# ZhenlongYuan/DVP-MVS

Measured on AMD Instinct MI355X. Metric: Mpixels/sec/PatchMatch-iteration, higher is better.
Workload: dtype f32

## Files before the change

__graft_entry__.py:

```python
import importlib
import os
import subprocess
import sys

ROOT = os.path.dirname(os.path.abspath(__file__))
if ROOT not in sys.path:
    sys.path.insert(0, ROOT)


def build() -> None:
    subprocess.check_call(["make", "-s", "-C", os.path.join(ROOT, "dvp-mvs_amd", "csrc")])
    host = os.path.join(ROOT, "dvp-mvs_amd", "host")
    if os.path.exists(os.path.join(host, "Makefile")):
        subprocess.check_call(["make", "-s", "-C", host])
    subprocess.check_call(["make", "-s", "-C", os.path.join(ROOT, "oracle")])
    subprocess.check_call(["make", "-s", "-C", os.path.join(ROOT, "tests", "emul")])
    subprocess.check_call(["make", "-s", "-C", os.path.join(ROOT, "tests", "host")])
    subprocess.check_call(["make", "-s", "-C", os.path.join(ROOT, "tests", "half16")])
    subprocess.check_call(["make", "-s", "-C", os.path.join(ROOT, "tests", "jpeg_host")])
    pkg = importlib.import_module("dvp-mvs_amd")
    lib = pkg.get_capi().lib()
    missing = [s for s in pkg.get_capi().EXPORTS if not hasattr(lib, s)]
    if missing:
        raise RuntimeError("libdvp_mvs_hip.so lacks symbols: %s" % missing)


def smoke() -> None:
    import numpy as np
    pkg = importlib.import_module("dvp-mvs_amd")
    synth, capi = pkg.synth, pkg.get_capi()
    from oracle import oracle as O
    W, H, S = 96, 64, 3
    sc = synth.make_scene(W, H, S)
    p = synth.default_params(S + 1, max_iterations=1, state=synth.FIRST_INIT, use_APD=0)
    p["depth_min"] = np.float32(2.5) * np.float32(0.6)
    p["depth_max"] = np.float32(6.5) * np.float32(1.2)
    state = dict(planes=np.zeros((H * W, 4), np.float32), edge=sc["edge"], label=sc["label"],
                 radius=np.full(H * W, 5, np.int32))
    g = capi.from_scene(sc, p, device=0)
    g.upload_state(**state)
    g.run_patchmatch()
    o = O.from_scene(sc, p)
    o.upload_state(**state)
    o.run_patchmatch()
    pg, po = g.get("planes"), o.get("planes")
    same = (pg.view(np.uint32) == po.view(np.uint32)) | (np.isnan(pg) & np.isnan(po))
    if not same.all():
        raise AssertionError("smoke: HIP planes differ from the oracle in %d values" % int((~same).sum()))
    for n in ("selected_views", "weak_info", "radius"):
# ... 10 lines not shown
```

dvp-mvs_amd/csrc/dvp_engine.hip:

```cpp
#include "dvp_stages.hpp"
#include "dvp_jpeg_enc.h"
#include <hip/hip_runtime.h>
#include <cstdlib>
#include <string>
#include <vector>
#include <cstdio>
#include <cstring>
#include <mutex>
#include <condition_variable>
#include <thread>
#include <chrono>
#include <algorithm>
#include <cmath>

using namespace dvp;

struct LaunchArgs {
	int tiles_x, tiles, rows, half, colour, iter;
};

template <int STAGE, int SMP, int MV = 32>
__device__ __forceinline__ void stage_body(const Dev& d, const LaunchArgs& a) {
	const int lane = threadIdx.x & 63;
	const int wave = threadIdx.x >> 6;
// ... 131 lines not shown
	}
	const int off = incl - n;
	const int total = __shfl(incl, 63, 64);
	{
		int k = 0;
		for (uint32_t m = uniq; m; m &= m - 1, ++k) items[off + k] = (uint8_t)lane;
	}
	__syncthreads();
	unsigned long long cnt = 0;
	for (int i0 = 0; i0 < total; i0 += 64) {
		const bool valid = i0 + lane < total;
		const int i = valid ? i0 + lane : total - 1;
		const int pl = items[i];
		const int k = i - __shfl(off, pl, 64);
		uint32_t m = (uint32_t)__shfl((int)uniq, pl, 64);
		for (int j = 0; j < k; ++j) m &= m - 1;
		const int slot = dvp_ctz(m);
		PatchCtx ci;
		ci.tab = PatchTab{&lds_tab[pl], 64};
		ci.sum_ref = __shfl(c.sum_ref, pl, 64);
		ci.sum_ref_ref = __shfl(c.sum_ref_ref, pl, 64);
		ci.wsum = __shfl(c.wsum, pl, 64);
		ci.radius = __shfl(c.radius, pl, 64);
		ci.inc = __shfl(c.inc, pl, 64);
		ci.fast = __shfl(c.fast, pl, 64);
		const int ipx = __shfl(px, pl, 64), ipy = __shfl(py, pl, 64);
		strong_eval_item<SMP>(d, ci, ipx, ipy, slot, valid, d.eval_counter ? &cnt : nullptr);
	}
	if (d.eval_counter && cnt) atomicAdd(d.eval_counter, cnt);
}
extern "C" __global__ void __launch_bounds__(64, DVP_LB_HEAVY) dvp_strong_eval_items(const Dev d, const LaunchArgs a) { strong_eval_items_body<0>(d, a); }
extern "C" __global__ void __launch_bounds__(64, DVP_LB_HEAVY) dvp_strong_eval_items_exact(const Dev d, const LaunchArgs a) { strong_eval_items_body<1>(d, a); }
DVP_KERNEL64(dvp_strong_refine, kStageStrongRefine, DVP_LB_HEAVY)
DVP_KERNEL64(dvp_strong_refine_lanes, kStageStrongRefineLanes, DVP_LB_HEAVY)
template <int MV>
__device__ __forceinline__ void strong_decide_body(const Dev& d, const LaunchArgs& a) {
	int px, py;
	if (!block_to_pixel(blockIdx.x, threadIdx.x & 63, threadIdx.x >> 6, a.tiles_x, a.tiles, a.rows, a.half, a.colour, d.width, d.height, &px, &py)) return;
	if (d.weak_info[px + py * d.width] != DVP_WEAK) strong_decide_px<MV>(d, px, py, a.iter);
}
#ifndef DVP_LB_DECIDE
#define DVP_LB_DECIDE 4
#endif
#define DVP_DECIDE_KERNEL(MV) extern "C" __global__ void __launch_bounds__(256, DVP_LB_DECIDE) dvp_strong_decide_v##MV(const Dev d, const LaunchArgs a) { strong_decide_body<MV>(d, a); }
DVP_DECIDE_KERNEL(4)
DVP_DECIDE_KERNEL(6)
DVP_DECIDE_KERNEL(8)
DVP_DECIDE_KERNEL(10)
DVP_DECIDE_KERNEL(12)
DVP_DECIDE_KERNEL(16)
DVP_KERNEL(dvp_get_depth_normal, DVP_ST_GET_DEPTH_NORMAL, 1)
DVP_KERNEL(dvp_filter_strong, DVP_ST_FILTER_STRONG, 1)
DVP_KERNEL(dvp_depth_to_weak, DVP_ST_DEPTH_TO_WEAK, DVP_LB_HEAVY)
DVP_KERNEL(dvp_local_refine, DVP_ST_LOCAL_REFINE, DVP_LB_HEAVY)
DVP_KERNEL(dvp_depth_to_weak_refine, kStageSweeps, DVP_LB_HEAVY)
template <int WHAT>
__device__ __forceinline__ void sweep_light_body(const Dev& d, const LaunchArgs& a) {
	int px, py;
	if (!block_to_pixel(blockIdx.x, threadIdx.x & 63, threadIdx.x >> 6, a.tiles_x, a.tiles, a.rows, 0, 0, d.width, d.height, &px, &py)) return;
	if (WHAT != 0 && d.sweep_row1 > 0 && (py < d.sweep_row0 || py >= d.sweep_row1)) return;
	if (WHAT == 0) sweep_prepare_px(d, px, py);
	else if (WHAT == 1) sweep_decide1_px(d, px, py);
	else sweep_decide2_px(d, px, py);
}
extern "C" __global__ void __launch_bounds__(256) dvp_sweep_prepare(const Dev d, const LaunchArgs a) { sweep_light_body<0>(d, a); }
extern "C" __global__ void __launch_bounds__(256) dvp_sweep_decide1(const Dev d, const LaunchArgs a) { sweep_light_body<1>(d, a); }
extern "C" __global__ void __launch_bounds__(256) dvp_sweep_decide2(const Dev d, const LaunchArgs a) { sweep_light_body<2>(d, a); }
// ... 744 lines not shown
	size_t L = 0;
	hipStream_t stream = nullptr;
	int cand_mask_mode = -1;
	bool cand_mask_on = true;
	uint8_t* cand_mask = nullptr;
	unsigned *cand_list = nullptr, *cand_n = nullptr;
	uint32_t* sel_snap = nullptr;
	hipStream_t side = nullptr;
	hipEvent_t side_fork = nullptr, side_join = nullptr;
	Dev d{};
	std::vector<void*> allocs;
	float* images = nullptr;
	uint8_t* images8 = nullptr;
	int* images8_flag = nullptr;
	bool images8_ok = false;
	bool no_images8 = false;
	uint32_t* images16 = nullptr;
	bool images16_ok = false;
	bool no_images16 = false;
	float* image_stage = nullptr;
	float* depths = nullptr;
	uint32_t* edge_bits = nullptr;
	uint32_t* strong_bits = nullptr;
	uint32_t* strong_bits_t = nullptr;
	int* edge_sat = nullptr;
	DvpCamera* cameras = nullptr; ViewConst* views = nullptr; int* sector_taps = nullptr; int* sector_start = nullptr;
	f4* planes = nullptr; f4* planes_snap = nullptr; f4* fit_planes = nullptr;
	int* search_pos = nullptr;
	float* slot_costs = nullptr;
	float* strong_rec = nullptr;
	bool strong_split = true;
	bool eval_items = true;
	bool refine_lanes = true;
	f4* sweep_rec = nullptr; float* sweep_cost = nullptr; float* sweep_pc = nullptr;
	bool ransac_wave = false;
	bool sweep_split = true;
	bool sweep_force = false;
	double sweep_band_gb = 0.0;
	int sweep_band_rows = 0;
	bool gn_wave = false;
	float* costs = nullptr; float* costs_snap = nullptr; float* complex_ = nullptr;
	uint32_t* selected_views = nullptr;
	uint8_t* view_weight = nullptr; uint8_t* weak_info = nullptr; uint8_t* weak_reliable = nullptr; uint8_t* edge = nullptr;
	s2* label_stop = nullptr; s2* weak_nearest_strong = nullptr; s2* neighbours = nullptr; s2* gn_points = nullptr; int* gn_count = nullptr; s2* candidate = nullptr; s2* edge_neigh = nullptr; s2* label_boundary = nullptr;
	int* neighbours_map = nullptr; int* label = nullptr; int* radius = nullptr;
	unsigned long long* eval_counter = nullptr;
	float* scratch_out = nullptr;
	size_t weak_alloc = 0;
	AnchorRec* anchor_tab = nullptr;
	size_t anchor_tab_alloc = 0;
	bool anchor_tab_valid = false;
	bool anchor_tab_off = false;
	WeakRec* weak_rec = nullptr; f2* weak_ctab = nullptr; float* weak_ev = nullptr;
	size_t weak_phase_alloc = 0;
	bool weak_phased = true;
	int weak_phased_min = 8192;
	int weak_run[4] = { 64, 256, 1024, 1024 };
	int weak_group[4] = { 1, 4, 4, 2 };
	int* weak_list = nullptr;
	size_t weak_list_alloc = 0;
	int* weak_counts = nullptr;
	int* weak_totals_host = nullptr;
	uint8_t* coarse = nullptr;
	uint8_t* maps_out = nullptr;
	hipStream_t copy = nullptr;
	uint8_t* maps_host = nullptr;
// ... 77 lines not shown

static int ensure_images16(dvp_ctx* c) {
	if (c->images16) return 0;
	return dalloc(c, &c->images16, img16_plane_bytes(c->W, c->H) / 4 * c->NI, false);
}

static int set_device(dvp_ctx* c) {
	HIP_TRY(c, hipSetDevice(c->device));
	return 0;
}

extern "C" {

int dvp_ctx_create(int device, int width, int height, int num_images, dvp_ctx** out) {
	if (!out) return 1;
	*out = nullptr;
	if (width <= 0 || height <= 0 || num_images < 2 || num_images > DVP_MAX_IMAGES || width > 32767 || height > 32767) {
		g_create_error = "dvp_ctx_create: bad dimensions (2 <= num_images <= 32, sizes <= 32767: short2 pixel coordinates)";
		return 1;
	}
	{
		const unsigned long long pitch = ((unsigned long long)width + 2 * kImgPad + 63) / 64 * 64;
		if (pitch * ((unsigned long long)height + 2 * kImgPad) * 8ull >= (1ull << 32)) {
			g_create_error = "dvp_ctx_create: image too large (a padded row-pair plane must stay below 4 GiB)";
			return 1;
		}
	}
	dvp_ctx* c = new dvp_ctx();
	c->device = device; c->W = width; c->H = height; c->NI = num_images;
	c->no_images8 = getenv("DVP_NO_IMAGES8") != nullptr;
	c->no_images16 = getenv("DVP_NO_IMAGES16") != nullptr;
	if (const char* e = getenv("DVP_STRONG_SPLIT")) c->strong_split = atoi(e) != 0;
	if (const char* e = getenv("DVP_REFINE_LANES")) c->refine_lanes = atoi(e) != 0;
	if (const char* e = getenv("DVP_EVAL_ITEMS")) c->eval_items = atoi(e) != 0;
	if (const char* e = getenv("DVP_SWEEP_SPLIT")) { c->sweep_split = atoi(e) != 0; c->sweep_force = atoi(e) == 2; }
	if (const char* e = getenv("DVP_SWEEP_BAND_GB")) c->sweep_band_gb = atof(e);
	if (const char* e = getenv("DVP_WEAK_ANCHOR_TAB")) c->anchor_tab_off = atoi(e) == 0;
	if (const char* e = getenv("DVP_GN_WAVE")) c->gn_wave = atoi(e) != 0;
	if (const char* e = getenv("DVP_RANSAC_WAVE")) c->ransac_wave = atoi(e) != 0;
	if (const char* e = getenv("DVP_CAND_MASK")) c->cand_mask_mode = atoi(e) != 0 ? 1 : 0;
	if (const char* e = getenv("DVP_WEAK_PHASED")) c->weak_phased = atoi(e) != 0;
	if (const char* e = getenv("DVP_WEAK_PHASED_MIN")) c->weak_phased_min = atoi(e);
	if (const char* e = getenv("DVP_WEAK_RUNS")) {
		int g[4];
		if (sscanf(e, "%d,%d,%d,%d", &g[0], &g[1], &g[2], &g[3]) == 4)
			for (int i = 0; i < 4; ++i) c->weak_run[i] = g[i] < 1 ? 1 : g[i];
	}
	if (const char* e = getenv("DVP_WEAK_GROUPS")) {
		int g[4];
		if (sscanf(e, "%d,%d,%d,%d", &g[0], &g[1], &g[2], &g[3]) == 4)
			for (int i = 0; i < 4; ++i) c->weak_group[i] = g[i] < 1 ? 1 : (g[i] > kGrp ? kGrp : g[i]);
	}
	c->pitch = (width + 2 * kImgPad + 63) / 64 * 64;
	c->L = (size_t)width * height;
	auto fail = [&](int) { g_create_error = c->error; dvp_ctx_destroy(c); return 1; };
	if (set_device(c)) return fail(0);
	if (hipStreamCreateWithFlags(&c->stream, hipStreamNonBlocking) != hipSuccess) { c->error = "hipStreamCreate failed"; return fail(0); }
	if (hipStreamCreateWithFlags(&c->side, hipStreamNonBlocking) != hipSuccess || hipEventCreateWithFlags(&c->side_fork, hipEventDisableTiming) != hipSuccess ||
	    hipEventCreateWithFlags(&c->side_join, hipEventDisableTiming) != hipSuccess) { c->error = "hipStreamCreate failed"; return fail(0); }
	const size_t L = c->L, S = (size_t)num_images - 1, plane = (size_t)c->pitch * (height + 2 * kImgPad);
	int r = 0;
	r |= dalloc(c, &c->images, plane * num_images * 2);
	r |= dalloc(c, &c->images8, (size_t)img8_tiles_x(width) * img8_tiles_y(height) * 128 * num_images);
	r |= dalloc(c, &c->images8_flag, (size_t)1);
	r |= dalloc(c, &c->image_stage, plane * num_images);
	r |= dalloc(c, &c->cameras, (size_t)num_images);
// ... 44 lines not shown
int dvp_ctx_destroy(dvp_ctx* c) {
	if (!c) return 0;
	(void)hipSetDevice(c->device);
	{
		int limit_s = 120;
		if (const char* e = getenv("DVP_DOWNLOAD_WAIT_S")) limit_s = atoi(e);
		std::unique_lock<std::mutex> lk(c->dl_m);
		c->dl_cv.wait_for(lk, std::chrono::seconds(limit_s > 0 ? limit_s : 1), [c] { return !c->dl_busy; });
		c->dl_cv.wait(lk, [c] { return !c->dl_fetching; });
	}
	if (c->copy) { (void)hipStreamSynchronize(c->copy); (void)hipStreamDestroy(c->copy); }
	if (c->pv_copy) { (void)hipStreamSynchronize(c->pv_copy); (void)hipStreamDestroy(c->pv_copy); }
	if (c->stream) (void)hipStreamSynchronize(c->stream);
	for (auto& e : c->pv_enc) dvpjpeg::encoder_free(e);
	if (c->pv_total) (void)hipHostFree(c->pv_total);
	if (c->pv_done) (void)hipEventDestroy(c->pv_done);
	if (c->maps_host) (void)hipHostFree(c->maps_host);
	if (c->stream) (void)hipStreamSynchronize(c->stream);
	for (auto& e : c->events) { (void)hipEventDestroy(e.a); (void)hipEventDestroy(e.b); }
	for (void* p : c->allocs) (void)hipFree(p);
	if (c->weak_totals_host) (void)hipHostFree(c->weak_totals_host);
	if (c->side) { (void)hipStreamSynchronize(c->side); (void)hipStreamDestroy(c->side); }
	if (c->side_fork) (void)hipEventDestroy(c->side_fork);
	if (c->side_join) (void)hipEventDestroy(c->side_join);
	if (c->stream) (void)hipStreamDestroy(c->stream);
	delete c;
	return 0;
}

#ifndef DVP_BUILD_ID
#define DVP_BUILD_ID "unknown"
#endif
const char* dvp_build_id(void) { return DVP_BUILD_ID; }

struct FinishError { const dvp_ctx* c = nullptr; std::string msg; };
static thread_local FinishError t_finish_error;
const char* dvp_last_error(const dvp_ctx* c) {
	if (c && t_finish_error.c == c && !t_finish_error.msg.empty()) return t_finish_error.msg.c_str();
	return c ? c->error.c_str() : g_create_error.c_str();
}

static int upload_planes(dvp_ctx* c, float* dst, const float* const* src, int pitch_floats, hipMemcpyKind kind, float* pairs = nullptr) {
	if (set_device(c)) return 1;
	if (pitch_floats < c->W) { c->error = "pitch_floats < width"; return 1; }
	const size_t stride = (size_t)c->pitch * (c->H + 2 * kImgPad);
	for (int i = 0; i < c->NI; ++i) {
		if (!src[i]) { c->error = "null image pointer"; return 1; }
		HIP_TRY(c, hipMemcpy2DAsync(dst + (size_t)i * stride + (size_t)kImgPad * c->pitch + kImgPad, (size_t)c->pitch * 4, src[i],
		                            (size_t)pitch_floats * 4, (size_t)c->W * 4, (size_t)c->H, kind, c->stream));
	}
	{
		const long long cells = (long long)(2 * kImgPad * (c->W + 2 * kImgPad) + 2 * kImgPad * c->H) * c->NI;
		hipLaunchKernelGGL(dvp_pad_replicate, dim3((unsigned)((cells + 255) / 256)), dim3(256), 0, c->stream, dst, c->W, c->H, c->pitch, stride, c->NI);
		HIP_TRY(c, hipGetLastError());
	}
	if (pairs) {
		const int PH = c->H + 2 * kImgPad;
		hipLaunchKernelGGL(dvp_interleave_rows, dim3((unsigned)((c->pitch + 255) / 256), (unsigned)PH, (unsigned)c->NI), dim3(256), 0, c->stream,
		                   dst, pairs, PH, c->pitch, stride, c->NI);
		HIP_TRY(c, hipGetLastError());
		HIP_TRY(c, hipMemsetAsync(c->images8_flag, 0, sizeof(int), c->stream));
		const int t8x = img8_tiles_x(c->W), t8y = img8_tiles_y(c->H);
		const size_t n = (size_t)t8x * t8y * 64 * c->NI;
		hipLaunchKernelGGL(dvp_pairs_to_tiles, dim3((unsigned)((n + 255) / 256)), dim3(256), 0, c->stream, pairs, c->images8, c->W + 2 * kImgPad, PH, c->pitch, stride,
		                   t8x, t8y, c->NI, c->images8_flag);
		HIP_TRY(c, hipGetLastError());
// ... 465 lines not shown
		HIP_TRY(c, hipGetLastError());
	}
	if (stage == DVP_ST_GEN_EDGE_INFORM && c->d.params.use_label && c->d.weak_count > 0) {
		if (!c->label_stop) {
			if (dalloc(c, &c->label_stop, c->L * 8, false)) return 1;
			sync_dev_struct(c);
		}
		hipLaunchKernelGGL(dvp_edge_rays, dim3((c->W + c->H + 255) / 256, 8), dim3(256), 0, c->stream, c->d, 1);
		HIP_TRY(c, hipGetLastError());
	}
	switch (stage) {
	case DVP_ST_GEN_EDGE_INFORM:
		if (!fused) {
			if (gen_candidates_all_views(c->d)) hipLaunchKernelGGL(dvp_gen_candidates_views, dim3(g.grid(), (unsigned)((c->NI - 1 + kCandGroup - 1) / kCandGroup)), block, 0, c->stream, c->d, a);
			else hipLaunchKernelGGL(dvp_gen_candidates, dim3(g.grid(), (unsigned)(c->NI - 1)), block, 0, c->stream, c->d, a);
		}
		hipLaunchKernelGGL(c->d.sampler ? dvp_gen_edge_inform_exact : dvp_gen_edge_inform, grid, block, 0, c->stream, c->d, a);
		break;
	case DVP_ST_RANDOM_INIT: hipLaunchKernelGGL(c->d.sampler ? dvp_random_init_exact : dvp_random_init, grid, block, 0, c->stream, c->d, a); break;
	case DVP_ST_STRONG_UPDATE:
		if (c->strong_split && c->NI - 1 <= 16) {
			ensure_strong_split_buffers(c);
		}
		if (c->strong_split && c->NI - 1 <= 16) {
			const int S = c->NI - 1;
			if (c->eval_items) hipLaunchKernelGGL(c->d.sampler ? dvp_strong_eval_items_exact : dvp_strong_eval_items, wave_grid, wave_block, 0, c->stream, c->d, a);
			else hipLaunchKernelGGL(c->d.sampler ? dvp_strong_eval_exact : dvp_strong_eval, wave_grid, wave_block, 0, c->stream, c->d, a);
			if (S <= 4) hipLaunchKernelGGL(dvp_strong_decide_v4, grid, block, 0, c->stream, c->d, a);
			else if (S <= 6) hipLaunchKernelGGL(dvp_strong_decide_v6, grid, block, 0, c->stream, c->d, a);
			else if (S <= 8) hipLaunchKernelGGL(dvp_strong_decide_v8, grid, block, 0, c->stream, c->d, a);
			else if (S <= 10) hipLaunchKernelGGL(dvp_strong_decide_v10, grid, block, 0, c->stream, c->d, a);
			else if (S <= 12) hipLaunchKernelGGL(dvp_strong_decide_v12, grid, block, 0, c->stream, c->d, a);
			else hipLaunchKernelGGL(dvp_strong_decide_v16, grid, block, 0, c->stream, c->d, a);
			if (c->refine_lanes && (size_t)c->pitch * (c->H + 2 * kImgPad) * 8 * c->NI < ((size_t)1 << 32))
				hipLaunchKernelGGL(c->d.sampler ? dvp_strong_refine_lanes_exact : dvp_strong_refine_lanes, wave_grid, wave_block, 0, c->stream, c->d, a);
			else hipLaunchKernelGGL(c->d.sampler ? dvp_strong_refine_exact : dvp_strong_refine, wave_grid, wave_block, 0, c->stream, c->d, a);
		}
		else if (c->NI - 1 <= kNarrowViews) hipLaunchKernelGGL(c->d.sampler ? dvp_strong_update_v8_exact : dvp_strong_update_v8, grid, block, 0, c->stream, c->d, a);
		else if (c->NI - 1 <= 16) hipLaunchKernelGGL(c->d.sampler ? dvp_strong_update_v16_exact : dvp_strong_update_v16, grid, block, 0, c->stream, c->d, a);
		else hipLaunchKernelGGL(c->d.sampler ? dvp_strong_update_exact : dvp_strong_update, grid, block, 0, c->stream, c->d, a);
		break;
	case DVP_ST_GET_DEPTH_NORMAL: hipLaunchKernelGGL(c->d.sampler ? dvp_get_depth_normal_exact : dvp_get_depth_normal, grid, block, 0, c->stream, c->d, a); break;
	case DVP_ST_FILTER_STRONG: hipLaunchKernelGGL(c->d.sampler ? dvp_filter_strong_exact : dvp_filter_strong, grid, block, 0, c->stream, c->d, a); break;
	case DVP_ST_DEPTH_TO_WEAK: {
		const bool sweep_passes = fused && c->sweep_split && (c->d.params.geom_consistency || c->sweep_force);
		if (sweep_passes) ensure_sweep_buffers(c);
		if (sweep_passes && c->sweep_split) {
			const bool ex = c->d.sampler != 0;
			LaunchArgs s0 = a, s1 = a, sb = a;
			s0.iter = 0; s1.iter = 1; sb.iter = kSweepBorderOnly;
			const int etx = (c->W + 63) / 64, ety = (c->H + kSweepRows - 1) / kSweepRows;
			s0.tiles_x = s1.tiles_x = etx; s0.tiles = s1.tiles = etx * ety;
			const dim3 egrid((unsigned)(etx * ety), (unsigned)(c->NI - 1));
			hipLaunchKernelGGL(dvp_sweep_prepare, grid, block, 0, c->stream, c->d, a);
			const int band_rows = c->sweep_band_rows > 0 ? c->sweep_band_rows : c->H;
			for (int row0 = 0; row0 < c->H; row0 += band_rows) {
				Dev db = c->d;
				LaunchArgs b0 = s0, b1 = s1;
				dim3 bgrid = egrid;
				b0.rows = b1.rows = 0;
				if (c->sweep_band_rows > 0) {
					const int row1 = std::min(c->H, row0 + band_rows);
					db.sweep_px0 = row0 * c->W; db.sweep_row0 = row0; db.sweep_row1 = row1;
					const int bty = (row1 - row0 + kSweepRows - 1) / kSweepRows;
					b0.rows = b1.rows = row0 / kSweepRows;
					b0.tiles = b1.tiles = etx * bty;
					bgrid = dim3((unsigned)(etx * bty), (unsigned)(c->NI - 1));
				}
// ... 479 lines not shown
```

dvp-mvs_amd/csrc/dvp_strong.hpp:

```cpp
#ifndef DVP_STRONG_HPP_
#define DVP_STRONG_HPP_

#include "dvp_ncc.hpp"

namespace dvp {

DVP_HD void sort_small(float* v, int n) {
	for (int i = 1; i < n; i++) {
		const float tmp = v[i];
		int j = i;
		for (; j >= 1 && tmp < v[j - 1]; j--) v[j] = v[j - 1];
		v[j] = tmp;
	}
}

DVP_HD f4 random_normal_yzl_sel(const Dev& d, int px, int py, Rng& rng, float depth, uint32_t sel) {
	const int W = d.width, H = d.height;
	const DvpCamera rc = load_camera(d, 0);
	f3 vd[20];
	{
		const f4 v0 = view_direction(rc, px, py, depth);
		vd[0] = mk3(v0.x, v0.y, v0.z);
	}
	int index = 1;
	for (int v = 1; v < d.params.num_images; ++v) {
		if (!is_set(sel, v - 1)) continue;
		const DvpCamera sc = load_camera(d, v);
		const f3 fwd = point_on_world((float)px, (float)py, depth, rc);
		f2 sp;
		float sd;
		project_on_camera(fwd, sc, &sp, &sd);
		const float sx = fminf(fmaxf(sp.x, -32768.0f), 32767.0f);
		const float sy = fminf(fmaxf(sp.y, -32768.0f), 32767.0f);
		const int ix = (int)((float)(int)sx + 0.5f), iy = (int)((float)(int)sy + 0.5f);
		float src_depth = 1.0f;
		if (d.params.geom_consistency) {
			if (ix >= 0 && ix < W && iy >= 0 && iy < H)
				src_depth = tex_texel(d.depths + (size_t)v * d.plane_stride, d.org, d.pitch, W, H, (int)sx, (int)sy);
// ... 749 lines not shown
		for (int k = 1; k < 8; ++k)
			if (k == min_cost_idx) { fmin = final_costs[k]; pmin = positions[k]; }
		if ((flag >> min_cost_idx) & 1) {
			const f4 cand = d.planes_snap[pmin];
			const float db = depth_from_plane(rc, cand, px, py);
			if (db >= P.depth_min && db <= P.depth_max && fmin < cost_now) {
				depth_now = db;
				plane_now = cand;
				cost_now = fmin;
				selected_views_written = true;
			}
		}
	}
	Rng rd(d.seed, (uint32_t)center, rng_site(PH_STRONG, iter, SUB_DEPTH_RAND));
	Rng rn(d.seed, (uint32_t)center, rng_site(PH_STRONG, iter, SUB_NORMAL));
	Rng rp(d.seed, (uint32_t)center, rng_site(PH_STRONG, iter, SUB_DEPTH_PERT));
	const float depth_rand = rd.uniform() * (P.depth_max - P.depth_min) + P.depth_min;
	if (selected_views_written) d.selected_views[center] = sel_mask;
#if defined(DVP_DECIDE_YZL_GENERIC)
	const f4 n_rand = random_normal_yzl(d, px, py, rn, depth_now);
#else
	const f4 n_rand = MV <= 16 ? random_normal_yzl_views<(MV <= 16 ? MV : 16)>(d, px, py, rn, depth_now, selected_views_written ? sel_mask : sel_entry)
	                           : random_normal_yzl(d, px, py, rn, depth_now);
#endif
	const float dmin_p = (1 - 0.02f) * depth_now, dmax_p = (1 + 0.02f) * depth_now;
	const float depth_pert = rp.uniform() * (dmax_p - dmin_p) + dmin_p;
	float* rec = d.strong_rec + hi;
	rec[(SR_PLANE + 0) * Lh] = plane_now.x; rec[(SR_PLANE + 1) * Lh] = plane_now.y; rec[(SR_PLANE + 2) * Lh] = plane_now.z; rec[(SR_PLANE + 3) * Lh] = plane_now.w;
	rec[SR_DEPTH * Lh] = depth_now; rec[SR_COST * Lh] = cost_now; rec[SR_CENTER * Lh] = costs_center;
	rec[SR_DRAND * Lh] = depth_rand; rec[SR_DPERT * Lh] = depth_pert;
	rec[(SR_NRAND + 0) * Lh] = n_rand.x; rec[(SR_NRAND + 1) * Lh] = n_rand.y; rec[(SR_NRAND + 2) * Lh] = n_rand.z;
}

template <int SMP, bool LANE_WALK = false>
DVP_HD void strong_refine_px(const Dev& d, int px, int py, PatchTab tab, unsigned long long* nevals) {
	const int W = d.width;
	const int center = py * W + px;
	const DvpParams& P = d.params;
	const DvpCamera rc = load_camera(d, 0);
	const int S = P.num_images - 1;
	const size_t Lh = (size_t)d.half_w * (size_t)d.height, hi = half_index(d, px, py);
	PatchCtx c;
	{
		int radius, inc;
		patch_geometry(d, center, &radius, &inc);
		build_patch_ctx(d, px, py, radius, inc, 0, tab, &c);
	}
	const float* rec = d.strong_rec + hi;
	f4 plane_now = mk4(rec[(SR_PLANE + 0) * Lh], rec[(SR_PLANE + 1) * Lh], rec[(SR_PLANE + 2) * Lh], rec[(SR_PLANE + 3) * Lh]);
	float depth_now = rec[SR_DEPTH * Lh], cost_now = rec[SR_COST * Lh], costs_center = rec[SR_CENTER * Lh];
	const float depth_rand = rec[SR_DRAND * Lh], depth_pert = rec[SR_DPERT * Lh];
	const f4 n_rand = mk4(rec[(SR_NRAND + 0) * Lh], rec[(SR_NRAND + 1) * Lh], rec[(SR_NRAND + 2) * Lh], 0.0f);
	f4 n_pert = plane_now;
	normalize3(&n_pert);
	const uint32_t* g32 = reinterpret_cast<const uint32_t*>(d.view_weight + (size_t)center * 32);
	uint32_t wq[8];
#pragma unroll
	for (int i = 0; i < 8; ++i) wq[i] = g32[i];
	float weight_norm = 0;
	for (int i = 0; i < S; ++i) {
		const int wv = (int)((wq[i >> 2] >> (8 * (i & 3))) & 255u);
		if (wv > 0) weight_norm += wv;
	}
	const float hyp_depth[5] = { depth_rand, depth_now, depth_rand, depth_now, depth_pert };
	const f4 hyp_normal[5] = { plane_now, n_rand, n_rand, n_pert, plane_now };
	const float depth_entry = depth_now;
	const f4 plane_entry = plane_now;
	(void)depth_entry; (void)plane_entry;
	if (LANE_WALK) {
		uint32_t sel = 0;
		for (int j = 0; j < S; ++j)
			if (((wq[j >> 2] >> (8 * (j & 3))) & 255u) > 0) sel |= 1u << j;
		int hyp = 0;
		bool busy = false;
		f4 plane = plane_now;
		float db = 0.0f, tc = 0.0f;
		uint32_t todo = 0;
		for (;;) {
			while (!busy && hyp < 5) {
				plane = hyp_normal[hyp];
				plane.w = distance_to_origin(rc, px, py, hyp_depth[hyp], plane);
				db = depth_from_plane(rc, plane, px, py);
				++hyp;
				if (!(db >= P.depth_min && db <= P.depth_max)) continue;
				if (!(weight_norm > 0.0f)) continue;
				tc = 0.0f;
				todo = sel;
				busy = true;
			}
			if (!busy) break;
			const int j = dvp_ctz(todo);
			todo &= todo - 1;
			uint32_t q = wq[0];
#pragma unroll
			for (int k = 1; k < 8; ++k) q = (j >> 2) == k ? wq[k] : q;
			const int wv = (int)((q >> (8 * (j & 3))) & 255u);
			tc += wv * ncc_old_lane<SMP>(d, c, px, py, j + 1, plane);
			if (nevals) *nevals += 1;
			const bool alive = tc / weight_norm < cost_now;
			if (!alive) busy = false;
			else if (todo == 0) {
				depth_now = db;
				plane_now = plane;
				cost_now = tc / weight_norm;
				busy = false;
			}
		}
	} else
	for (int i = 0; i < 5; ++i) {
		f4 plane = hyp_normal[i];
		plane.w = distance_to_origin(rc, px, py, hyp_depth[i], plane);
		const float db = depth_from_plane(rc, plane, px, py);
		if (!(db >= P.depth_min && db <= P.depth_max)) continue;
		float tc = 0.0f;
		bool alive = weight_norm > 0.0f;
		for (int j = 0; j < S && alive; ++j) {
			const int wv = (int)((wq[j >> 2] >> (8 * (j & 3))) & 255u);
			if (wv > 0) {
				tc += wv * ncc_old<SMP>(d, c, px, py, j + 1, plane);
				if (nevals) *nevals += 1;
				alive = tc / weight_norm < cost_now;
			}
		}
		if (alive) {
			depth_now = db;
			plane_now = plane;
			cost_now = tc / weight_norm;
		}
	}
	if (P.state == DVP_REFINE_INIT) {
		if (cost_now < costs_center - 0.1) {
			costs_center = cost_now;
			d.planes[center] = plane_now;
		}
	} else {
		costs_center = cost_now;
		d.planes[center] = plane_now;
	}
	d.costs[center] = costs_center;
}

DVP_HD void get_depth_normal_px(const Dev& d, int px, int py) {
	const int center = py * d.width + px;
	f4 pl = d.planes[center];
	pl.w = depth_from_plane(d.cameras[0], pl, px, py);
	d.planes[center] = normal_cam_to_world(d.cameras[0], pl);
}

DVP_HD void filter_strong_px(const Dev& d, int px, int py) {
	const int W = d.width, H = d.height;
	const int center = py * W + px;
	if (d.costs[center] < 0.001f) return;
	float filter[21];
	int n = 0;
	filter[n++] = d.planes[center].w;
	const int ox[20] = { 0, 0, 0, 0, 0, 0, -1, -3, -5, 1, 3, 5, 2, 2, -2, -2, -1, 1, -1, 1 };
	const int oy[20] = { -1, -3, -5, 1, 3, 5, 0, 0, 0, 0, 0, 0, -1, 1, -1, 1, -2, -2, 2, 2 };
	for (int t = 0; t < 20; ++t) {
		const int x = px + ox[t], y = py + oy[t];
		if (x < 0 || y < 0 || x >= W || y >= H) continue;
		if (oy[t] == -2 && py <= 2) continue;
		const int q = x + y * W;
		if (d.weak_info[q] == DVP_STRONG) filter[n++] = d.planes[q].w;
	}
	sort_small(filter, n);
	const int m = n / 2;
	d.planes[center].w = (n % 2 == 0) ? (filter[m - 1] + filter[m]) / 2 : filter[m];
}

struct SweepCtx {
	f4 origin;
	float depth;
// ... 589 lines not shown
```

dvp-mvs_amd/csrc/dvp_weak_wave.hpp:

```cpp
#ifndef DVP_WEAK_WAVE_HPP_
#define DVP_WEAK_WAVE_HPP_

#include "dvp_weak.hpp"

#if defined(DVP_GN_STATS) && !defined(__HIPCC__)
#include <cstdio>
#endif
namespace dvp {

#if defined(__HIP_DEVICE_COMPILE__)
#define DVP_LANES(L) for (int L = (int)(threadIdx.x & 63u), once_##L = 1; once_##L; once_##L = 0)
#define DVP_LANE0 ((threadIdx.x & 63u) == 0u)
DVP_HD void wave_sync() {
	__builtin_amdgcn_fence(__ATOMIC_RELEASE, "wavefront");
	__builtin_amdgcn_wave_barrier();
	__builtin_amdgcn_fence(__ATOMIC_ACQUIRE, "wavefront");
}
#else
#define DVP_LANES(L) for (int L = 0; L < 64; ++L)
#define DVP_LANE0 true
DVP_HD void wave_sync() {}
#endif

constexpr int kAnchors = DVP_NEIGHBOUR_NUM - 1;
constexpr int kAnchorTaps = kAnchors * 9;
#ifndef DVP_WEAK_PAIRS
#define DVP_WEAK_PAIRS 40
#endif
constexpr int kWeakPairs = DVP_WEAK_PAIRS;
constexpr int kWeakViews = 7;

template <int TAB>
struct WeakSharedT {
	f2 ctab[kTaps * kTaps];
	float caa[kTaps * kTaps];
	float rows[kWeakPairs][kTaps][3];
	float acost[kWeakPairs][kAnchors];
	int inq[kWeakPairs];
	uint32_t aoff[TAB ? 1 : kWeakViews * kAnchors][4];
	uint8_t astate[kWeakViews * kAnchors];
	union {
		float cost_array[8][32];
		float Hq[TAB ? kWeakPairs : 1][9];
	};
	float ev[8][32];
	float gtab[8][32];
	float probs[32];
	float priors[32];
	float fcost[8];
	int positions[8];
	uint8_t vw[32];
	f4 pl[8];
};
using WeakShared = WeakSharedT<0>;

// ... 1691 lines not shown
```

Measured before the change: 59.71.

## Add phased wave-cooperative strong refine kernel with compacted hypothesis chains

Replaces the per-lane hypothesis walk in strong refine with a wave-level phased scheme. Each round compacts the still-alive (pixel, hypothesis) chains into LDS and redistributes NCC evaluations across all 64 lanes, optionally evaluating 2 or 4 views per chain in later rounds. The aim is to remove the divergence and idle lanes of the per-lane early-exit walk. In exchange it adds LDS traffic, shuffles and per-round synchronisation, and may evaluate a few views past the point where a chain would have been pruned. The old walk kernel stays available behind an environment flag, and optional stats counters are added.

```diff
diff --git a/__graft_entry__.py b/__graft_entry__.py
--- a/__graft_entry__.py
+++ b/__graft_entry__.py
@@ -15,6 +15,7 @@
         subprocess.check_call(["make", "-s", "-C", host])
     subprocess.check_call(["make", "-s", "-C", os.path.join(ROOT, "oracle")])
     subprocess.check_call(["make", "-s", "-C", os.path.join(ROOT, "tests", "emul")])
+    subprocess.check_call(["make", "-s", "-C", os.path.join(ROOT, "tests", "emul_refine")])
     subprocess.check_call(["make", "-s", "-C", os.path.join(ROOT, "tests", "host")])
     subprocess.check_call(["make", "-s", "-C", os.path.join(ROOT, "tests", "half16")])
     subprocess.check_call(["make", "-s", "-C", os.path.join(ROOT, "tests", "jpeg_host")])
diff --git a/dvp-mvs_amd/csrc/dvp_engine.hip b/dvp-mvs_amd/csrc/dvp_engine.hip
--- a/dvp-mvs_amd/csrc/dvp_engine.hip
+++ b/dvp-mvs_amd/csrc/dvp_engine.hip
@@ -187,7 +187,26 @@
 extern "C" __global__ void __launch_bounds__(64, DVP_LB_HEAVY) dvp_strong_eval_items(const Dev d, const LaunchArgs a) { strong_eval_items_body<0>(d, a); }
 extern "C" __global__ void __launch_bounds__(64, DVP_LB_HEAVY) dvp_strong_eval_items_exact(const Dev d, const LaunchArgs a) { strong_eval_items_body<1>(d, a); }
 DVP_KERNEL64(dvp_strong_refine, kStageStrongRefine, DVP_LB_HEAVY)
-DVP_KERNEL64(dvp_strong_refine_lanes, kStageStrongRefineLanes, DVP_LB_HEAVY)
+DVP_KERNEL64(dvp_strong_refine_walk, kStageStrongRefineLanes, DVP_LB_HEAVY)
+template <int SMP>
+__device__ __forceinline__ void strong_refine_wave_body(const Dev& d, const LaunchArgs& a) {
+	const int lane = threadIdx.x;
+	const int b = blockIdx.x;
+	const int tile = (b >> 5) * 8 + (b & 7), wave = (b >> 3) & 3;
+	__shared__ f2 lds_tab[kTaps * kTaps * 64];
+	__shared__ RefineShared sh;
+	static_assert(sizeof(RefineShared) <= 2048, "18 KB table + 2 KB: eight workgroups per CU");
+	int px = 0, py = 0;
+	bool active = block_to_pixel(tile, lane, wave, a.tiles_x, a.tiles, a.rows, a.half, a.colour, d.width, d.height, &px, &py);
+	if (active && d.weak_info[px + py * d.width] == DVP_WEAK) active = false;
+	LaneVar<int> pxy;
+	pxy.at(lane) = active ? (px | (py << 16)) : -1;
+	unsigned long long n = 0;
+	strong_refine_wave<SMP>(d, pxy, lds_tab, sh, d.eval_counter ? &n : nullptr);
+	if (d.eval_counter && n) atomicAdd(d.eval_counter, n);
+}
+extern "C" __global__ void __launch_bounds__(64, DVP_LB_HEAVY) dvp_strong_refine_lanes(const Dev d, const LaunchArgs a) { strong_refine_wave_body<0>(d, a); }
+extern "C" __global__ void __launch_bounds__(64, DVP_LB_HEAVY) dvp_strong_refine_lanes_exact(const Dev d, const LaunchArgs a) { strong_refine_wave_body<1>(d, a); }
 template <int MV>
 __device__ __forceinline__ void strong_decide_body(const Dev& d, const LaunchArgs& a) {
 	int px, py;
@@ -998,6 +1017,7 @@
 	bool strong_split = true;
 	bool eval_items = true;
 	bool refine_lanes = true;
+	bool refine_phased = true;
 	f4* sweep_rec = nullptr; float* sweep_cost = nullptr; float* sweep_pc = nullptr;
 	bool ransac_wave = false;
 	bool sweep_split = true;
@@ -1141,6 +1161,7 @@
 	c->no_images16 = getenv("DVP_NO_IMAGES16") != nullptr;
 	if (const char* e = getenv("DVP_STRONG_SPLIT")) c->strong_split = atoi(e) != 0;
 	if (const char* e = getenv("DVP_REFINE_LANES")) c->refine_lanes = atoi(e) != 0;
+	if (const char* e = getenv("DVP_REFINE_PHASED")) c->refine_phased = atoi(e) != 0;
 	if (const char* e = getenv("DVP_EVAL_ITEMS")) c->eval_items = atoi(e) != 0;
 	if (const char* e = getenv("DVP_SWEEP_SPLIT")) { c->sweep_split = atoi(e) != 0; c->sweep_force = atoi(e) == 2; }
 	if (const char* e = getenv("DVP_SWEEP_BAND_GB")) c->sweep_band_gb = atof(e);
@@ -1251,6 +1272,14 @@
 #define DVP_BUILD_ID "unknown"
 #endif
 const char* dvp_build_id(void) { return DVP_BUILD_ID; }
+#if defined(DVP_REFINE_STATS)
+extern "C" int dvp_refine_stats(unsigned long long* out) {
+	unsigned long long zero[8] = {};
+	if (hipDeviceSynchronize() != hipSuccess) return 1;
+	if (hipMemcpyFromSymbol(out, HIP_SYMBOL(g_refine_stats), sizeof(zero)) != hipSuccess) return 1;
+	return hipMemcpyToSymbol(HIP_SYMBOL(g_refine_stats), zero, sizeof(zero)) != hipSuccess;
+}
+#endif
 
 struct FinishError { const dvp_ctx* c = nullptr; std::string msg; };
 static thread_local FinishError t_finish_error;
@@ -1782,8 +1811,10 @@
 			else if (S <= 10) hipLaunchKernelGGL(dvp_strong_decide_v10, grid, block, 0, c->stream, c->d, a);
 			else if (S <= 12) hipLaunchKernelGGL(dvp_strong_decide_v12, grid, block, 0, c->stream, c->d, a);
 			else hipLaunchKernelGGL(dvp_strong_decide_v16, grid, block, 0, c->stream, c->d, a);
-			if (c->refine_lanes && (size_t)c->pitch * (c->H + 2 * kImgPad) * 8 * c->NI < ((size_t)1 << 32))
-				hipLaunchKernelGGL(c->d.sampler ? dvp_strong_refine_lanes_exact : dvp_strong_refine_lanes, wave_grid, wave_block, 0, c->stream, c->d, a);
+			if (c->refine_lanes && (size_t)c->pitch * (c->H + 2 * kImgPad) * 8 * c->NI < ((size_t)1 << 32)) {
+				if (c->refine_phased) hipLaunchKernelGGL(c->d.sampler ? dvp_strong_refine_lanes_exact : dvp_strong_refine_lanes, wave_grid, wave_block, 0, c->stream, c->d, a);
+				else hipLaunchKernelGGL(c->d.sampler ? dvp_strong_refine_walk_exact : dvp_strong_refine_walk, wave_grid, wave_block, 0, c->stream, c->d, a);
+			}
 			else hipLaunchKernelGGL(c->d.sampler ? dvp_strong_refine_exact : dvp_strong_refine, wave_grid, wave_block, 0, c->stream, c->d, a);
 		}
 		else if (c->NI - 1 <= kNarrowViews) hipLaunchKernelGGL(c->d.sampler ? dvp_strong_update_v8_exact : dvp_strong_update_v8, grid, block, 0, c->stream, c->d, a);
diff --git a/dvp-mvs_amd/csrc/dvp_strong.hpp b/dvp-mvs_amd/csrc/dvp_strong.hpp
--- a/dvp-mvs_amd/csrc/dvp_strong.hpp
+++ b/dvp-mvs_amd/csrc/dvp_strong.hpp
@@ -4,6 +4,47 @@
 #include "dvp_ncc.hpp"
 
 namespace dvp {
+
+#if defined(__HIP_DEVICE_COMPILE__)
+#define DVP_LANES(L) for (int L = (int)(threadIdx.x & 63u), once_##L = 1; once_##L; once_##L = 0)
+#define DVP_LANE0 ((threadIdx.x & 63u) == 0u)
+DVP_HD void wave_sync() {
+	__builtin_amdgcn_fence(__ATOMIC_RELEASE, "wavefront");
+	__builtin_amdgcn_wave_barrier();
+	__builtin_amdgcn_fence(__ATOMIC_ACQUIRE, "wavefront");
+}
+#else
+#if defined(DVP_LANES_REVERSE)
+#define DVP_LANES(L) for (int L = 63; L >= 0; --L)
+#else
+#define DVP_LANES(L) for (int L = 0; L < 64; ++L)
+#endif
+#define DVP_LANE0 true
+DVP_HD void wave_sync() {}
+#endif
+template <class T>
+struct LaneVar {
+#if defined(__HIP_DEVICE_COMPILE__)
+	T v;
+	DVP_HD T& at(int) { return v; }
+	DVP_HD T at(int) const { return v; }
+	DVP_HD T from(int src) const { return __shfl(v, src, 64); }
+#else
+	T v[64];
+	DVP_HD T& at(int l) { return v[l]; }
+	DVP_HD T at(int l) const { return v[l]; }
+	DVP_HD T from(int src) const { return v[src]; }
+#endif
+};
+DVP_HD unsigned long long lane_ballot_bit(const LaneVar<uint32_t>& m, int bit) {
+#if defined(__HIP_DEVICE_COMPILE__)
+	return __ballot((int)((m.v >> bit) & 1u));
+#else
+	unsigned long long r = 0;
+	for (int l = 0; l < 64; ++l) r |= (unsigned long long)((m.v[l] >> bit) & 1u) << l;
+	return r;
+#endif
+}
 
 DVP_HD void sort_small(float* v, int n) {
 	for (int i = 1; i < n; i++) {
@@ -819,6 +860,15 @@
 	rec[(SR_NRAND + 0) * Lh] = n_rand.x; rec[(SR_NRAND + 1) * Lh] = n_rand.y; rec[(SR_NRAND + 2) * Lh] = n_rand.z;
 }
 
+#if defined(DVP_REFINE_STATS) && defined(__HIPCC__)
+__device__ unsigned long long g_refine_stats[8];
+#endif
+DVP_HD void refine_stats_add(int which, unsigned long long n) {
+#if defined(DVP_REFINE_STATS) && defined(__HIP_DEVICE_COMPILE__)
+	atomicAdd(&g_refine_stats[which], n);
+#endif
+}
+
 template <int SMP, bool LANE_WALK = false>
 DVP_HD void strong_refine_px(const Dev& d, int px, int py, PatchTab tab, unsigned long long* nevals) {
 	const int W = d.width;
@@ -863,6 +913,9 @@
 		f4 plane = plane_now;
 		float db = 0.0f, tc = 0.0f;
 		uint32_t todo = 0;
+#if defined(DVP_REFINE_STATS) && defined(__HIP_DEVICE_COMPILE__)
+		int stat_trips = 0;
+#endif
 		for (;;) {
 			while (!busy && hyp < 5) {
 				plane = hyp_normal[hyp];
@@ -875,6 +928,17 @@
 				todo = sel;
 				busy = true;
 			}
+#if defined(DVP_REFINE_STATS) && defined(__HIP_DEVICE_COMPILE__)
+			{
+				const unsigned long long still = __ballot(busy ? 1 : 0);
+				if (!busy) {
+					if (still == 0ull && (int)(threadIdx.x & 63u) == (int)__builtin_ctzll(__ballot(1))) { refine_stats_add(0, 1); refine_stats_add(1, (unsigned long long)stat_trips); }
+					refine_stats_add(2, (unsigned long long)stat_trips);
+					refine_stats_add(3, 1);
+				}
+			}
+			if (busy) ++stat_trips;
+#endif
 			if (!busy) break;
 			const int j = dvp_ctz(todo);
 			todo &= todo - 1;
@@ -925,6 +989,213 @@
 		d.planes[center] = plane_now;
 	}
 	d.costs[center] = costs_center;
+}
+
+#ifndef DVP_REFINE_GROUP_FROM
+#define DVP_REFINE_GROUP_FROM 2
+#endif
+struct RefineShared {
+	float tc[5 * 64];
+	uint16_t chain[5 * 64];
+};
+DVP_HD f4 refine_hypothesis(const DvpCamera& rc, int px, int py, int h, const f4 plane_now, const f4 n_rand, float depth_rand, float depth_now, float depth_pert) {
+	f4 plane = plane_now;
+	if (h == 1 || h == 2) plane = n_rand;
+	if (h == 3) normalize3(&plane);
+	const float depth = (h == 0 || h == 2) ? depth_rand : (h == 4 ? depth_pert : depth_now);
+	plane.w = distance_to_origin(rc, px, py, depth, plane);
+	return plane;
+}
+template <int SMP>
+DVP_HD void strong_refine_wave(const Dev& d, const LaneVar<int>& pxy ,
+	f2* tab , RefineShared& sh, unsigned long long* nevals) {
+	const DvpParams& P = d.params;
+	const DvpCamera rc = load_camera(d, 0);
+	const int S = P.num_images - 1;
+	const size_t Lh = (size_t)d.half_w * (size_t)d.height;
+	LaneVar<float> sum_ref, sum_ref_ref, wsum, cost_entry, wnorm, pnx, pny, pnz, rnx, rny, rnz, d_rand, d_now, d_pert;
+	LaneVar<int> radius, inc;
+	LaneVar<uint32_t> selfast;
+	LaneVar<uint32_t> wlo, whi;
+	LaneVar<uint32_t> chains, live;
+	DVP_LANES(l) {
+		sum_ref.at(l) = sum_ref_ref.at(l) = wsum.at(l) = cost_entry.at(l) = wnorm.at(l) = 0.0f;
+		pnx.at(l) = pny.at(l) = pnz.at(l) = rnx.at(l) = rny.at(l) = rnz.at(l) = d_rand.at(l) = d_now.at(l) = d_pert.at(l) = 0.0f;
+		radius.at(l) = inc.at(l) = 0;
+		selfast.at(l) = wlo.at(l) = whi.at(l) = chains.at(l) = live.at(l) = 0u;
+#pragma unroll
+		for (int h = 0; h < 5; ++h) sh.tc[h * 64 + l] = 0.0f;
+		if (pxy.at(l) < 0) continue;
+		const int px = pxy.at(l) & 0xFFFF, py = pxy.at(l) >> 16;
+		const int center = py * d.width + px;
+		PatchCtx c;
+		c.sum_ref = c.sum_ref_ref = c.wsum = 0.0f;
+		{
+			int r, s;
+			patch_geometry(d, center, &r, &s);
+			build_patch_ctx(d, px, py, r, s, 0, PatchTab{tab + l, 64}, &c);
+		}
+		sum_ref.at(l) = c.sum_ref; sum_ref_ref.at(l) = c.sum_ref_ref; wsum.at(l) = c.wsum;
+		radius.at(l) = c.radius; inc.at(l) = c.inc;
+		const float* rec = d.strong_rec + half_index(d, px, py);
+		const f4 plane_now = mk4(rec[(SR_PLANE + 0) * Lh], rec[(SR_PLANE + 1) * Lh], rec[(SR_PLANE + 2) * Lh], rec[(SR_PLANE + 3) * Lh]);
+		const f4 n_rand = mk4(rec[(SR_NRAND + 0) * Lh], rec[(SR_NRAND + 1) * Lh], rec[(SR_NRAND + 2) * Lh], 0.0f);
+		pnx.at(l) = plane_now.x; pny.at(l) = plane_now.y; pnz.at(l) = plane_now.z;
+		rnx.at(l) = n_rand.x; rny.at(l) = n_rand.y; rnz.at(l) = n_rand.z;
+		d_rand.at(l) = rec[SR_DRAND * Lh]; d_now.at(l) = rec[SR_DEPTH * Lh]; d_pert.at(l) = rec[SR_DPERT * Lh];
+		cost_entry.at(l) = rec[SR_COST * Lh];
+		const uint32_t* g32 = reinterpret_cast<const uint32_t*>(d.view_weight + (size_t)center * 32);
+		uint32_t wq[4];
+#pragma unroll
+		for (int i = 0; i < 4; ++i) wq[i] = g32[i];
+		float weight_norm = 0;
+		uint32_t sel = 0, lo = 0, hi = 0;
+		for (int i = 0; i < S; ++i) {
+			const int wv = (int)((wq[i >> 2] >> (8 * (i & 3))) & 255u);
+			if (wv > 0) {
+				weight_norm += wv;
+				sel |= 1u << i;
+				if (i < 8) lo |= (uint32_t)wv << (4 * i); else hi |= (uint32_t)wv << (4 * (i - 8));
+			}
+		}
+		wnorm.at(l) = weight_norm;
+		selfast.at(l) = sel | (c.fast ? 0x10000u : 0u);
+		wlo.at(l) = lo; whi.at(l) = hi;
+		uint32_t m = 0;
+		if (weight_norm > 0.0f) {
+#pragma unroll
+			for (int h = 0; h < 5; ++h) {
+				const f4 plane = refine_hypothesis(rc, px, py, h, plane_now, n_rand, d_rand.at(l), d_now.at(l), d_pert.at(l));
+				const float db = depth_from_plane(rc, plane, px, py);
+				if (db >= P.depth_min && db <= P.depth_max) m |= 1u << h;
+			}
+		}
+		chains.at(l) = m;
+	}
+	wave_sync();
+	unsigned long long cnt = 0, stat_trips = 0, stat_rounds = 0;
+	for (int k0 = 0; k0 < S;) {
+		DVP_LANES(l) {
+			uint32_t m = k0 == 0 ? chains.at(l) : live.at(l);
+#pragma unroll
+			for (int h = 0; h < 5; ++h)
+				if (((m >> h) & 1u) && !(sh.tc[h * 64 + l] < INFINITY)) m &= ~(1u << h);
+			if (k0 >= __builtin_popcount(selfast.at(l) & 0xFFFFu)) m = 0;
+			live.at(l) = m;
+		}
+		int n = 0;
+		for (int h = 0; h < 5; ++h) {
+			const unsigned long long b = lane_ballot_bit(live, h);
+			DVP_LANES(l) {
+				if ((b >> l) & 1ull) sh.chain[n + __builtin_popcountll(b & ((1ull << l) - 1ull))] = (uint16_t)(l | (h << 6));
+			}
+			n += __builtin_popcountll(b);
+		}
+		if (n == 0) break;
+		wave_sync();
+		int m = 1;
+		if (k0 >= DVP_REFINE_GROUP_FROM) {
+			const int t1 = ((n + 63) >> 6) * 4, t2 = ((2 * n + 63) >> 6) * 2, t4 = (4 * n + 63) >> 6;
+			if (t2 < t1) m = 2;
+			if (t4 < t1 && t4 < t2) m = 4;
+		}
+		const int sm = m == 4 ? 2 : (m == 2 ? 1 : 0);
+		++stat_rounds;
+		for (int i0 = 0; i0 < n * m; i0 += 64) {
+			++stat_trips;
+			LaneVar<float> prod, it_wn, it_ce;
+			LaneVar<int> it_chain, it_nv;
+			DVP_LANES(l) {
+				const int s = i0 + l;
+				const int sub = s & (m - 1);
+				const bool have = (s >> sm) < n;
+				const int e = sh.chain[have ? (s >> sm) : n - 1];
+				const int p = e & 63, h = e >> 6;
+				const uint32_t sf = selfast.from(p);
+				const int nv = __builtin_popcount(sf & 0xFFFFu);
+				const bool valid = have && k0 + sub < nv;
+				const int kk = k0 + sub < nv ? k0 + sub : nv - 1;
+				uint32_t vm = sf & 0xFFFFu;
+				for (int q = 0; q < kk; ++q) vm &= vm - 1;
+				const int j = dvp_ctz(vm);
+				const uint32_t lo = wlo.from(p), hi = whi.from(p);
+				const int wv = (int)(((j < 8 ? lo : hi) >> (4 * (j & 7))) & 15u);
+				PatchCtx ci;
+				ci.tab = PatchTab{tab + p, 64};
+				ci.sum_ref = sum_ref.from(p); ci.sum_ref_ref = sum_ref_ref.from(p); ci.wsum = wsum.from(p);
+				ci.radius = radius.from(p); ci.inc = inc.from(p); ci.fast = (int)((sf >> 16) & 1u);
+				const int ip = pxy.from(p);
+				const int ipx = ip & 0xFFFF, ipy = ip >> 16;
+				const f4 plane_now = mk4(pnx.from(p), pny.from(p), pnz.from(p), 0.0f);
+				const f4 n_rand = mk4(rnx.from(p), rny.from(p), rnz.from(p), 0.0f);
+				const float dr = d_rand.from(p), dn = d_now.from(p), dp = d_pert.from(p);
+				it_wn.at(l) = wnorm.from(p);
+				it_ce.at(l) = cost_entry.from(p);
+				it_nv.at(l) = nv;
+				it_chain.at(l) = (have && sub == 0) ? e : -1;
+				prod.at(l) = 0.0f;
+#if !defined(__HIP_DEVICE_COMPILE__)
+				if (!valid) continue;
+#endif
+				const f4 plane = refine_hypothesis(rc, ipx, ipy, h, plane_now, n_rand, dr, dn, dp);
+				prod.at(l) = wv * ncc_old_lane<SMP>(d, ci, ipx, ipy, j + 1, plane);
+				if (valid) ++cnt;
+			}
+			DVP_LANES(l) {
+				float c4[4];
+#pragma unroll
+				for (int q = 0; q < 4; ++q) c4[q] = q < m ? prod.from((l + q) & 63) : 0.0f;
+				const int e = it_chain.at(l);
+				if (e < 0) continue;
+				float t = sh.tc[(e >> 6) * 64 + (e & 63)];
+#pragma unroll
+				for (int q = 0; q < 4; ++q) {
+					if (q < m && k0 + q < it_nv.at(l) && t < INFINITY) {
+						t += c4[q];
+						if (!(t / it_wn.at(l) < it_ce.at(l))) t = INFINITY;
+					}
+				}
+				sh.tc[(e >> 6) * 64 + (e & 63)] = t;
+			}
+		}
+		wave_sync();
+		k0 += m;
+	}
+	if (nevals) *nevals += cnt;
+	if (DVP_LANE0) { refine_stats_add(0, 1); refine_stats_add(1, stat_trips); refine_stats_add(4, stat_rounds); }
+	DVP_LANES(l) {
+		refine_stats_add(2, cnt);
+		if (pxy.at(l) < 0) continue;
+		refine_stats_add(3, 1);
+		const int px = pxy.at(l) & 0xFFFF, py = pxy.at(l) >> 16;
+		const int center = py * d.width + px;
+		const float* rec = d.strong_rec + half_index(d, px, py);
+		const f4 plane_entry = mk4(pnx.at(l), pny.at(l), pnz.at(l), rec[(SR_PLANE + 3) * Lh]);
+		const f4 n_rand = mk4(rnx.at(l), rny.at(l), rnz.at(l), 0.0f);
+		f4 plane_now = plane_entry;
+		float cost_now = cost_entry.at(l), costs_center = rec[SR_CENTER * Lh];
+#pragma unroll
+		for (int h = 0; h < 5; ++h) {
+			if (!((chains.at(l) >> h) & 1u)) continue;
+			const float t = sh.tc[h * 64 + l];
+			if (!(t < INFINITY)) continue;
+			const float cost = t / wnorm.at(l);
+			if (cost < cost_now) {
+				plane_now = refine_hypothesis(rc, px, py, h, plane_entry, n_rand, d_rand.at(l), d_now.at(l), d_pert.at(l));
+				cost_now = cost;
+			}
+		}
+		if (P.state == DVP_REFINE_INIT) {
+			if (cost_now < costs_center - 0.1) {
+				costs_center = cost_now;
+				d.planes[center] = plane_now;
+			}
+		} else {
+			costs_center = cost_now;
+			d.planes[center] = plane_now;
+		}
+		d.costs[center] = costs_center;
+	}
 }
 
 DVP_HD void get_depth_normal_px(const Dev& d, int px, int py) {
diff --git a/dvp-mvs_amd/csrc/dvp_weak_wave.hpp b/dvp-mvs_amd/csrc/dvp_weak_wave.hpp
--- a/dvp-mvs_amd/csrc/dvp_weak_wave.hpp
+++ b/dvp-mvs_amd/csrc/dvp_weak_wave.hpp
@@ -8,19 +8,6 @@
 #endif
 namespace dvp {
 
-#if defined(__HIP_DEVICE_COMPILE__)
-#define DVP_LANES(L) for (int L = (int)(threadIdx.x & 63u), once_##L = 1; once_##L; once_##L = 0)
-#define DVP_LANE0 ((threadIdx.x & 63u) == 0u)
-DVP_HD void wave_sync() {
-	__builtin_amdgcn_fence(__ATOMIC_RELEASE, "wavefront");
-	__builtin_amdgcn_wave_barrier();
-	__builtin_amdgcn_fence(__ATOMIC_ACQUIRE, "wavefront");
-}
-#else
-#define DVP_LANES(L) for (int L = 0; L < 64; ++L)
-#define DVP_LANE0 true
-DVP_HD void wave_sync() {}
-#endif
 
 constexpr int kAnchors = DVP_NEIGHBOUR_NUM - 1;
 constexpr int kAnchorTaps = kAnchors * 9;
```

Result: no change. 60.26 (median of 6 runs) (+0.9%).
